# Black-Phoenix/CUDA-SfM

Hardware: AMD Instinct MI355X
Metric: RANSAC E-matrix hypotheses/sec (8-point, fused scoring), inlier-mask parity vs CPU oracle (higher is better)
Workload: dtype f32

## Files before the change

cuda-sfm_amd/csrc/ransac_prefilter.hip:

```cpp
#include "ransac_device.hpp"
#include "block_ops.hpp"
#include "prefilter_math.hpp"
#include "prefilter_record.hpp"
#include "prefilter_lds.hpp"

namespace sfm {

typedef float f16v __attribute__((ext_vector_type(16)));


__device__ constexpr int kPfESlot[9] = { 2, 6, 1, 3, 5, 7, 0, 4, 8 };
__device__ __forceinline__ uint32_t shift_in_reject(uint32_t rejected, float nt, float G)
{
    return __builtin_amdgcn_alignbit(rejected, __float_as_uint(fmaf(-nt, nt, G)), 31);
}

__device__ __forceinline__ uint32_t scan16(const f16v &nt, const f16v &G)
{
    uint32_t rejected = 0u;
#pragma unroll
    for (int r = 0; r < 16; ++r) rejected = shift_in_reject(rejected, nt[r], G[r]);
    return rejected;
}

// ... 16 lines not shown
    const uint32_t wb = pf_bfi(kPackM0 | kPackM1, pf_bfi(kPackM0, d[3], d[4]), d[5]);
    return pf_bfi(0x55555555u, wa, wb << 1);
}

typedef uint32_t u2v __attribute__((ext_vector_type(2)));
typedef float f4v __attribute__((ext_vector_type(4)));
typedef __attribute__((address_space(3))) u2v lds_u2;
typedef uint32_t u4v __attribute__((ext_vector_type(4)));
typedef __attribute__((address_space(3))) u4v lds_u4;
typedef __attribute__((address_space(3))) const f4v lds_cf4;
typedef __attribute__((address_space(3))) const float lds_cf;
typedef __attribute__((address_space(3))) int lds_i;
typedef __attribute__((address_space(3))) const h8 lds_ch8;
typedef __attribute__((address_space(3))) const v2f lds_cv2;
typedef __attribute__((address_space(3))) const unsigned char lds_cu8;

struct PfFrags { h8 n0, n1, t; };

__device__ __forceinline__ bool pf_exact_inlier(v2f p0, v2f p1, v2f p2, v2f p3, float e8, v2f xu, v2f yv, const ThrBand &band)
{
    const v2f e00 = { p3.x, p3.x }, e44 = { p3.y, p3.y }, e31 = { p1.y, p1.x };
    const v2f ab0 = __builtin_elementwise_fma(p1, yv, __builtin_elementwise_fma(e00, xu, p0));
    const v2f ab1 = __builtin_elementwise_fma(e44, yv, __builtin_elementwise_fma(e31, xu, p2));
    const float a2 = fmaf(p2.y, yv.x, fmaf(p0.y, xu.x, e8));
    const float nn = fmaf(yv.y, ab1.x, fmaf(xu.y, ab0.x, a2));
    const float n2 = nn * nn;
    const v2f dd = __builtin_elementwise_fma(ab1, ab1, ab0 * ab0);
    const float da = dd.x, db = dd.y;
    const float m = n2 * (da + db);
    const float tp = (da * db) * band.thr;
    const uint32_t mb = __float_as_uint(m), tb = __float_as_uint(tp);
    const uint32_t gap = __usad(mb, tb, 0u);
    const bool undecided = (gap < kBandUlps) || (tb < band.lo_bits) || (tb > band.hi_bits);
    bool in = m < tp;
    if (undecided) {
        const float t1 = (da == 0.0f) ? 0.0f : n2 / da;
        const float t2 = (db == 0.0f) ? 0.0f : n2 / db;
        in = (t1 + t2) < band.thr;
    }
    return in;
}

template <int RULE>
__device__ __forceinline__ PfFrags load_point_frags(lds_ch8 *frag_lane, int pb)
{
    lds_ch8 *p = frag_lane + pb * (PfLds<RULE>::kBlockBytes / 16);
    if (RULE != kPfRuleG) return PfFrags{ p[0], p[64], h8{} };
    return PfFrags{ p[0], p[64], p[128] };
}

template <int RULE>
__device__ __forceinline__ void mfma_step(const PfFrags &a, const PfFrags &b, f16v &G, f16v &nt)
{
    const f16v z = {};
    nt = __builtin_amdgcn_mfma_f32_32x32x16_f16(a.n0, b.n0, z, 0, 0, 0);
    if (RULE == kPfRuleG) G = __builtin_amdgcn_mfma_f32_32x32x16_f16(a.t, b.t, z, 0, 0, 0);
    nt = __builtin_amdgcn_mfma_f32_32x32x16_f16(a.n1, b.n1, nt, 0, 0, 0);
}

#define PF_SCHED_STEP()                                                 \
    do {                                                                \
        if (RULE != kPfRuleG) {                                         \
            __builtin_amdgcn_sched_group_barrier(0x008, 1, 0);          \
            __builtin_amdgcn_sched_group_barrier(0x002, 8, 0);          \
            __builtin_amdgcn_sched_group_barrier(0x008, 1, 0);          \
            __builtin_amdgcn_sched_group_barrier(0x002, 8, 0);          \
        } else {                                                        \
            __builtin_amdgcn_sched_group_barrier(0x008, 1, 0);          \
            __builtin_amdgcn_sched_group_barrier(0x002, 11, 0);         \
            __builtin_amdgcn_sched_group_barrier(0x008, 1, 0);          \
            __builtin_amdgcn_sched_group_barrier(0x002, 11, 0);         \
            __builtin_amdgcn_sched_group_barrier(0x008, 1, 0);          \
            __builtin_amdgcn_sched_group_barrier(0x002, 11, 0);         \
        }                                                               \
    } while (0)

constexpr int kPfVarTickets = 1;
constexpr int kPfVarDrainLocal = 2;
constexpr int kPfVarClosedDecode = 4;
constexpr int kPfVarAnswerEpilogue = 8;
constexpr int kPfVarDrainK1 = 16, kPfVarDrainK7 = 32;
constexpr int kPfVarSinglePass = 64;
constexpr int kPfVarPairDrain = 128;

constexpr int pf_score_waves_per_simd(int var, int rule, int fl2, int pipe, int wide, int prio)
{
    if ((var == 0 || var == kPfVarPairDrain) && rule == kPfRuleBandTile && !fl2 && !pipe && !wide && !prio) return 4;
    return ((var & kPfVarTickets) == 0 && (rule == kPfRuleBandTile || rule == kPfRuleBandPack) && !fl2 && !pipe && !wide && !prio) ? 5 : 4;
}

template <int W, int VAR = 0, int RULE = kPfRuleBandTile, int FL2 = 0, int PIPE = 0, int WIDE = 0, int PRIO = 0>
__global__ __launch_bounds__(W * 64, pf_score_waves_per_simd(VAR, RULE, FL2, PIPE, WIDE, PRIO))
void ransac_score_prefilter(const float *__restrict__ X0, const float *__restrict__ X1, int ld, int n,
                            const float *__restrict__ Ecand, const PfRecord *__restrict__ recs, uint32_t h0, uint32_t count, float thr,
                            int dynamic, int tile,
                            int *__restrict__ counts, uint32_t *__restrict__ tick,
                            unsigned long long *best_key, unsigned long long *best_key2, unsigned long long *__restrict__ clk,
                            const unsigned long long *__restrict__ bound_word, const uint32_t *__restrict__ tile_boxes)
{
    extern __shared__ __attribute__((aligned(16))) unsigned char smem[];
    const int lane = threadIdx.x & 63;
    const int wave = __builtin_amdgcn_readfirstlane(threadIdx.x >> 6);
    const bool probe = clk && blockIdx.x == 0 && blockIdx.y == 0 && threadIdx.x == 0;
    unsigned long long c0 = 0, w0 = 0;
    if (clk && blockIdx.x == 0 && blockIdx.y == 0 && wave == 0) { c0 = clock64(); w0 = wall_clock64(); }
#if SFM_AB
    const uint32_t trace_blk = blockIdx.y * gridDim.x + blockIdx.x;
    unsigned long long *trace = (clk && trace_blk < (uint32_t)kTraceBlocks) ? clk + 8 + (size_t)trace_blk * kTraceWords : nullptr;
    if (trace && threadIdx.x == 0) {
        trace[0] = wall_clock64();
        trace[2] = ((unsigned long long)__builtin_amdgcn_s_getreg((20 << 0) | (0 << 6) | (31 << 11)) << 32) |
                   (unsigned long long)__builtin_amdgcn_s_getreg((4 << 0) | (0 << 6) | (31 << 11));
        trace[3] = ((unsigned long long)blockIdx.y << 32) | blockIdx.x;
    }
#define PF_PHASE(k) do { if (probe1) clk[k] = wall_clock64() - w0; } while (0)
#else
#define PF_PHASE(k) do { } while (0)
#endif
    const int half = lane >> 5, row = lane & 31;
    uint32_t npass = (count + (uint32_t)kPfGroup - 1u) / (uint32_t)kPfGroup;
    const uint32_t nstatic = gridDim.x * (uint32_t)W;
    using LT = PfLds<RULE>;
    constexpr bool kBand = RULE != kPfRuleG, kTile = RULE == kPfRuleBandTile, kPack = RULE == kPfRuleBandPack || kTile;
    static_assert(!(FL2 && kPack) && !((VAR & kPfVarTickets) && kPack), "the recorded variants were built on the v_alignbit scan");
    constexpr bool kTail9 = kPack && W == 16 && !FL2 && !PIPE && !WIDE && !PRIO && !(VAR & kPfVarTickets);
    static_assert(kTail9 || (VAR & ~kPfVarTickets) == 0, "the pass-tail switches belong to the product's two rules");
    static_assert(!(VAR & kPfVarSinglePass) || (kTile && VAR == kPfVarSinglePass), "single passes: the per-tile rule's summing instance");
    static_assert(!(VAR & kPfVarPairDrain) || (kTile && VAR == kPfVarPairDrain), "paired passes drained between the scans: the per-tile rule's summing instance");
    constexpr bool kPair = kTile && kTail9 && (VAR == 0 || VAR == kPfVarPairDrain);
    constexpr bool kCarry = kPair && VAR == 0;
    constexpr int kRows = kPair ? kPfPairRows : kPfPassRows, kUnit = kRows;
    constexpr int kDrainMore = !kTail9 ? 0 : (VAR & kPfVarDrainK1) ? 1 : (VAR & kPfVarDrainK7) ? 7 : (VAR & kPfVarDrainLocal) ? 3 : 0;
    constexpr bool kDecodeTable = !(kTail9 && (VAR & kPfVarClosedDecode));
    constexpr bool kSumCounts = kTail9 && !(VAR & kPfVarAnswerEpilogue);
    constexpr int kRing = FL2 ? 256 : kPfRing;
    constexpr int kEnt = WIDE ? 16 : 8;
    static_assert(!WIDE || (kPack && !PIPE && !FL2), "wide entries: the packed scan's plain loop only");
    if (kPair) npass = (npass + 1u) >> 1;
    const LT L(tile, kRing, kEnt, kRows);
    float *etab = reinterpret_cast<float *>(smem + L.wave + wave * pf_wave_bytes(kRows));
    int *cnt = reinterpret_cast<int *>(etab + kRows * kPfERow);

    PfFrags afrag = {};
    h8 bfrag_n0 = {}, bfrag_n1 = {};
    uint32_t key0 = 0u;
    float rec_dn = 0.0f, rec_lin = 0.0f;
    float e_row[9] = {};
    auto fetch_pass = [&](uint32_t pass, PfFrags &af, uint32_t &k0, float (&e)[9], float &dn, float &lin) {
        const uint32_t hf = pass * (uint32_t)kUnit;
        const uint32_t h = hf + (uint32_t)min(kPair ? lane : row, (int)min((uint32_t)kUnit, count - hf) - 1);
        if (kTile) {
            const float *src = Ecand + 9 * (size_t)h;
#pragma unroll
            for (int k = 0; k < 9; ++k) e[k] = src[k];
            const uint4 rec = reinterpret_cast<const uint4 *>(recs)[h];
            k0 = rec.x; dn = __uint_as_float(rec.y); lin = __uint_as_float(rec.z);
            return;
        }
        const uint4 *r = reinterpret_cast<const uint4 *>(recs + h) + 2 * half;
        const uint4 r0 = r[0], r1 = r[1];
        if (kBand) pf_band_record_expand(r0, r1, half, af.n0, af.n1, k0);
        else pf_record_expand(r0, r1, half, af.n0, af.n1, af.t, k0);
        if (half == 0) {
            const float *src = Ecand + 9 * (size_t)h;
#pragma unroll
            for (int k = 0; k < 9; ++k) e[k] = src[k];
        }
    };
    auto install_rows = [&](const float (&e)[9]) {
        if (kPair || half == 0) {
            const int r = kPair ? lane : row;
#pragma unroll
            for (int k = 0; k < 9; ++k) etab[kRows * k + r] = e[kPfESlot[k]];
            cnt[r] = 0;
        }
    };
    uint32_t ps = blockIdx.x * (uint32_t)W + (uint32_t)wave;
    bool have = ps < npass;
    if (have) { fetch_pass(ps, afrag, key0, e_row, rec_dn, rec_lin); install_rows(e_row); }

    SFM_PHASE("stage_tile");
    uint32_t *next_idx = reinterpret_cast<uint32_t *>(smem + L.next);
    if (threadIdx.x == 0) *next_idx = (uint32_t)W;
    if constexpr (kCarry) {
        if (threadIdx.x < kPfRingLutBytes) smem[L.lut + threadIdx.x] = (unsigned char)pf_ring_lut_entry(threadIdx.x);
    } else
    if (kPack && kDecodeTable && threadIdx.x < 32) smem[L.lut + threadIdx.x] = (unsigned char)pf_pack_code((int)threadIdx.x);
    float pf_B = 0.0f;
    uint32_t bw[8] = {};
    uint32_t bw_lane = 0u;
    if (kTile) {
        pf_B = __uint_as_float((uint32_t)(__hip_atomic_load(reinterpret_cast<const uint32_t *>(bound_word), __ATOMIC_RELAXED, __HIP_MEMORY_SCOPE_AGENT)));
        bw_lane = __hip_atomic_load(tile_boxes + 8 * blockIdx.y + (lane & 7), __ATOMIC_RELAXED, __HIP_MEMORY_SCOPE_AGENT);
    }
    __syncthreads();
    const int tile_first = blockIdx.y * tile;
    for (int t = threadIdx.x; t < L.staged; t += W * 64) {
        const int p = tile_first + t;
        float u = 0.f, v = 0.f, x = 0.f, y = 0.f;
        const bool real = p < n && t < tile;
        if (kTile) {
            if (real) {
                const float4 q4 = reinterpret_cast<const float4 *>(X0)[p];
                u = q4.x; v = q4.y; x = q4.z; y = q4.w;
            }
        } else
        if (real) { u = X0[p]; v = X0[(size_t)ld + p]; x = X1[p]; y = X1[(size_t)ld + p]; }
        _Float16 bn[kPfSlots], bt[kPfSlotsT];
        prefilter_point_slots(u, v, x, y, real, bn, bt);
        reinterpret_cast<float4 *>(smem + L.pts)[t] = real ? make_float4(x, u, y, v) : make_float4(NAN, NAN, NAN, NAN);
        const int pb = t >> 5, col = t & 31;
        unsigned char *blk = smem + LT::kFrag + pb * LT::kBlockBytes;
#pragma unroll
        for (int ks = 0; ks < 2; ++ks)
#pragma unroll
            for (int hh = 0; hh < 2; ++hh) {
                h8 c;
#pragma unroll
                for (int j = 0; j < 8; ++j) c[j] = bn[ks * 16 + hh * 8 + j];
                *reinterpret_cast<h8 *>(blk + ks * 1024 + (hh * 32 + col) * 16) = c;
            }
        if (RULE == kPfRuleG) {
#pragma unroll
            for (int hh = 0; hh < 2; ++hh) {
                h8 c;
#pragma unroll
                for (int j = 0; j < 8; ++j) c[j] = bt[hh * 8 + j];
                *reinterpret_cast<h8 *>(blk + 2048 + (hh * 32 + col) * 16) = c;
            }
        }
    }
    __syncthreads();
    PfBox tbox = {};
    auto build_operands = [&](const float (&e)[9], uint32_t fl, float dn, float lin) {
        int half_l = half;
        float thr_l = thr, B_l = pf_B;
        asm volatile("" : "+v"(half_l), "+s"(thr_l), "+s"(B_l));
        key0 = fl & kPfTileFlagScan;
        if constexpr (kPair) {
            h8 x0, y0, x1, y1;
            pf_tile_operands_full(e, fl, dn, lin, thr_l, B_l, tbox, x0, y0, x1, y1);
            u4v xa = __builtin_bit_cast(u4v, x0), ya = __builtin_bit_cast(u4v, y0), xb = __builtin_bit_cast(u4v, x1), yb = __builtin_bit_cast(u4v, y1);
#pragma unroll
            for (int w = 0; w < 4; ++w) {
                const u2v sa = __builtin_amdgcn_permlane32_swap(xa[w], ya[w], false, false);
                const u2v sb = __builtin_amdgcn_permlane32_swap(xb[w], yb[w], false, false);
                xa[w] = sa.x; ya[w] = sa.y; xb[w] = sb.x; yb[w] = sb.y;
            }
            afrag.n0 = __builtin_bit_cast(h8, xa); afrag.n1 = __builtin_bit_cast(h8, xb);
            bfrag_n0 = __builtin_bit_cast(h8, ya); bfrag_n1 = __builtin_bit_cast(h8, yb);
        } else
        pf_tile_operands(e, fl, dn, lin, thr_l, B_l, tbox, half_l, afrag.n0, afrag.n1);
    };
    if (kTile) {
#pragma unroll
        for (int k = 0; k < 8; ++k) bw[k] = (uint32_t)__builtin_amdgcn_readlane((int)bw_lane, k);
        pf_B = uniform(pf_B);
        tbox = pf_box_from_bits(bw, pf_B);
        tbox = PfBox{ uniform(tbox.xlo), uniform(tbox.xhi), uniform(tbox.ylo), uniform(tbox.yhi), uniform(tbox.ulo), uniform(tbox.uhi), uniform(tbox.vlo), uniform(tbox.vhi) };
        if (have) build_operands(e_row, key0, rec_dn, rec_lin);
    }
#if SFM_AB
    if (probe) clk[2] = wall_clock64() - w0;
#endif
    const int npb = (min(tile, ld - tile_first) + 31) >> 5;
    const int npp = (npb + 1) >> 1;
    const float4 *pts = reinterpret_cast<const float4 *>(smem + L.pts);
    lds_cf *etab_l = (lds_cf *)etab;
    lds_i *cnt_l = (lds_i *)cnt;
    lds_cu8 *lut_l = (lds_cu8 *)(smem + L.lut);
    const uint32_t ring_base = (uint32_t)(size_t)(__attribute__((address_space(3))) unsigned char *)(smem + L.ring) + (uint32_t)wave * (uint32_t)(kRing * kEnt);
    uint32_t ring_mask = (uint32_t)(kRing * kEnt - 1);
    asm("" : "+v"(ring_mask));
    auto ring_at = [&](uint32_t index8) {
        return (lds_u2 *)((__attribute__((address_space(3))) unsigned char *)0 + ((index8 & ring_mask) | ring_base));
    };
    auto ring_at16 = [&](uint32_t index16) {
        return (lds_u4 *)((__attribute__((address_space(3))) unsigned char *)0 + ((index16 & ring_mask) | ring_base));
    };
    lds_ch8 *frag_lane = (lds_ch8 *)(smem + LT::kFrag) + lane;
    const ThrBand band = make_band(thr);
    uint32_t passes_done = 0;
#if SFM_AB
    uint32_t carried = 0;
#endif

    while (have) {
        SFM_PHASE("pass_begin");
        const uint32_t h_first = ps * (uint32_t)kUnit;
        const int nvalid_unit = (int)min((uint32_t)kUnit, count - h_first);
        int nvalid = min(nvalid_unit, kPfGroup), hoff = 0;
        const int nscan = (kPair && nvalid_unit > kPfGroup) ? 2 : 1;
#if SFM_AB
        const bool probe1 = probe && passes_done == 0u;
        unsigned long long w_scan_end = 0;
#endif
        uint32_t ps_next = ps + nstatic;
        if (dynamic) {
            uint32_t got = 0u;
            if (lane == 0) got = atomicAdd(next_idx, 1u);
            got = (uint32_t)__builtin_amdgcn_readfirstlane((int)got);
            ps_next = (got / (uint32_t)W) * nstatic + blockIdx.x * (uint32_t)W + (got % (uint32_t)W);
        }
        const unsigned long long scan_rows = __ballot(key0 != 0u);
        int head = 0, nq = 0;
        auto patch_zero_divisor_rows = [&](int sc) {
            uint32_t todo = kPair ? (uint32_t)(sc ? scan_rows >> 32 : scan_rows) : ((uint32_t)scan_rows | (uint32_t)(scan_rows >> 32));
            uint32_t survive = 0u;
            while (todo) {
                const int r = __builtin_ctz(todo) + hoff;
                todo &= todo - 1u;
                const float se[6] = { etab[6 * kRows + r], etab[2 * kRows + r], etab[r], etab[3 * kRows + r], etab[7 * kRows + r], etab[4 * kRows + r] };
                bool z = false;
                for (int j = 0; j < L.staged / 64; ++j) {
                    const float4 q = pts[j * 64 + lane];
                    z = z || prefilter_zero_divisor(se, q.x, q.z);
                }
                if (__ballot(z) != 0ull) survive |= 1u << (r - hoff);
            }
            if (survive != 0u && ((survive >> row) & 1u)) {
                const h8 zero = {};
                afrag.n0 = zero; afrag.n1 = zero; afrag.t = zero;
                if (half) { afrag.n1[3] = (_Float16)1.0f; afrag.t[7] = (_Float16)0.0009765625f; }
            }
        };

        uint32_t lane_tag = (uint32_t)(size_t)(lds_cf4 *)pts + (uint32_t)(row * 16) + (uint32_t)(half * 4);
        auto decide_first = [&](uint32_t &rest, uint32_t tag) {
            const int b = __builtin_clz(rest);
            rest &= ~(0x80000000u >> b);
            int hl, sub;
            if constexpr (kCarry) {
                const uint32_t code = (uint32_t)lut_l[pf_ring_lut_index(b, tag)];
                hl = (int)(code & 63u); sub = (int)(code >> 6);
            } else if (kPack) {
                const uint32_t code = kDecodeTable ? (uint32_t)lut_l[b] : pf_pack_code_closed(b);
                hl = (int)(code & 31u) + (int)(tag & 4u); sub = (int)(code >> 5);
            } else {
                const int r = kBand ? b >> 1 : b & 15;
                sub = kBand ? b & 1 : b >> 4;
                hl = r + (r & 12) + (int)(tag & 4u);
            }
            const int row_end = kCarry ? nvalid_unit : nvalid, row_first = kCarry ? 0 : hoff;
            if (hl < row_end) {
                const f4v q = *(lds_cf4 *)((__attribute__((address_space(3))) const unsigned char *)0 + ((tag & ~15u) + ((uint32_t)sub << 9)));
                lds_cf *e = etab_l + hl + row_first;
                const v2f p0 = { e[0], e[kRows] }, p1 = { e[2 * kRows], e[3 * kRows] }, p2 = { e[4 * kRows], e[5 * kRows] }, p3 = { e[6 * kRows], e[7 * kRows] };
                const float e8 = e[8 * kRows];
                if (pf_exact_inlier(p0, p1, p2, p3, e8, v2f{ q.x, q.y }, v2f{ q.z, q.w }, band))
                    __hip_atomic_fetch_add(cnt_l + hl + row_first, 1, __ATOMIC_RELAXED, __HIP_MEMORY_SCOPE_WORKGROUP);
            }
        };
        auto flush = [&](int m, auto more_c) {
            constexpr int kMore = decltype(more_c)::value;
            uint32_t rest = 0, tag = 0;
            if (PRIO == 2) __builtin_amdgcn_s_setprio(2);
            if (lane < m) {
                const u2v ent = *ring_at(((uint32_t)head + (uint32_t)lane) * 8u);
                tag = ent.y;
                rest = ent.x;
                decide_first(rest, tag);
                if constexpr (kMore > 0) {
#pragma unroll 1
                    for (int it = 0; it < kMore && rest != 0u; ++it) decide_first(rest, tag);
                }
            }
            const unsigned long long more = __ballot(rest != 0u);
            if (more) {
                const int slot = __builtin_amdgcn_mbcnt_hi((uint32_t)(more >> 32), __builtin_amdgcn_mbcnt_lo((uint32_t)more, 0u));
                if (rest) *ring_at(((uint32_t)(head + nq) + (uint32_t)slot) * 8u) = u2v{ rest, tag };
            }
            head = (head + m) & (kRing - 1);
            nq += __builtin_popcountll(more) - m;
            if (PRIO == 2) __builtin_amdgcn_s_setprio(0);
        };
        constexpr std::integral_constant<int, 0> kInLoop{};
        constexpr std::integral_constant<int, kDrainMore> kDrain{};
        auto flush_w = [&](int m) {
            uint32_t ra = 0, rb = 0, tag = 0;
            if (lane < m) {
                const u4v ent = *ring_at16(((uint32_t)head + (uint32_t)lane) * 16u);
                tag = ent.z;
                const bool second = ent.x == 0u;
                const uint32_t surv = second ? ent.y : ent.x;
                const int b = __builtin_clz(surv);
                const uint32_t left = surv & ~(0x80000000u >> b);
                ra = second ? 0u : left; rb = second ? left : ent.y;
                const uint32_t code = lut_l[b];
                const int hl = (int)(code & 31u) + (int)(tag & 4u);
                if (hl < nvalid) {
                    const f4v q = *(lds_cf4 *)((__attribute__((address_space(3))) const unsigned char *)0 + ((tag & ~15u) + ((code >> 5) << 9) + (second ? 1024u : 0u)));
                    lds_cf *e = etab_l + hl;
                    const v2f p0 = { e[0], e[32] }, p1 = { e[64], e[96] }, p2 = { e[128], e[160] }, p3 = { e[192], e[224] };
                    const float e8 = e[256];
                    if (pf_exact_inlier(p0, p1, p2, p3, e8, v2f{ q.x, q.y }, v2f{ q.z, q.w }, band))
                        __hip_atomic_fetch_add(cnt_l + hl, 1, __ATOMIC_RELAXED, __HIP_MEMORY_SCOPE_WORKGROUP);
                }
            }
            const unsigned long long more = __ballot((ra | rb) != 0u);
            if (more) {
                const int slot = __builtin_amdgcn_mbcnt_hi((uint32_t)(more >> 32), __builtin_amdgcn_mbcnt_lo((uint32_t)more, 0u));
                if ((ra | rb) != 0u) *ring_at16(((uint32_t)(head + nq) + (uint32_t)slot) * 16u) = u4v{ ra, rb, tag, 0u };
            }
            head = (head + m) & (kRing - 1);
            nq += __builtin_popcountll(more) - m;
        };
        auto flush2 = [&]() {
            const u2v entA = *ring_at(((uint32_t)head + (uint32_t)lane) * 8u), entB = *ring_at(((uint32_t)head + 64u + (uint32_t)lane) * 8u);
            const int bA = __builtin_clz(entA.x), bB = __builtin_clz(entB.x);
            const uint32_t restA = entA.x & ~(0x80000000u >> bA), restB = entB.x & ~(0x80000000u >> bB);
            const int rA = bA >> 1, rB = bB >> 1;
            const int hlA = rA + (rA & 12) + (int)(entA.y & 4u), hlB = rB + (rB & 12) + (int)(entB.y & 4u);
            const int hcA = min(hlA, nvalid - 1), hcB = min(hlB, nvalid - 1);
            const f4v qA = *(lds_cf4 *)((__attribute__((address_space(3))) const unsigned char *)0 + ((entA.y & ~15u) + ((uint32_t)(bA & 1) << 9)));
            const f4v qB = *(lds_cf4 *)((__attribute__((address_space(3))) const unsigned char *)0 + ((entB.y & ~15u) + ((uint32_t)(bB & 1) << 9)));
            lds_cf *eA = etab_l + hcA, *eB = etab_l + hcB;
            const v2f a0 = { eA[0], eA[32] }, a1 = { eA[64], eA[96] }, a2 = { eA[128], eA[160] }, a3 = { eA[192], eA[224] };
            const float a8 = eA[256];
            const v2f b0 = { eB[0], eB[32] }, b1 = { eB[64], eB[96] }, b2 = { eB[128], eB[160] }, b3 = { eB[192], eB[224] };
            const float b8 = eB[256];
            const bool inA = pf_exact_inlier(a0, a1, a2, a3, a8, v2f{ qA.x, qA.y }, v2f{ qA.z, qA.w }, band);
            const bool inB = pf_exact_inlier(b0, b1, b2, b3, b8, v2f{ qB.x, qB.y }, v2f{ qB.z, qB.w }, band);
            if (inA && hlA < nvalid) __hip_atomic_fetch_add(cnt_l + hlA, 1, __ATOMIC_RELAXED, __HIP_MEMORY_SCOPE_WORKGROUP);
            if (inB && hlB < nvalid) __hip_atomic_fetch_add(cnt_l + hlB, 1, __ATOMIC_RELAXED, __HIP_MEMORY_SCOPE_WORKGROUP);
            const unsigned long long moreA = __ballot(restA != 0u), moreB = __ballot(restB != 0u);
            if (moreA | moreB) {
                const int nA = __builtin_popcountll(moreA);
                const int slotA = __builtin_amdgcn_mbcnt_hi((uint32_t)(moreA >> 32), __builtin_amdgcn_mbcnt_lo((uint32_t)moreA, 0u));
                const int slotB = nA + __builtin_amdgcn_mbcnt_hi((uint32_t)(moreB >> 32), __builtin_amdgcn_mbcnt_lo((uint32_t)moreB, 0u));
                if (restA) *ring_at(((uint32_t)(head + nq) + (uint32_t)slotA) * 8u) = u2v{ restA, entA.y };
                if (restB) *ring_at(((uint32_t)(head + nq) + (uint32_t)slotB) * 8u) = u2v{ restB, entB.y };
            }
            head = (head + 128) & (kRing - 1);
            nq += __builtin_popcountll(moreA) + __builtin_popcountll(moreB) - 128;
        };

        for (int sc = 0; ; ++sc) {
        patch_zero_divisor_rows(sc);
#if SFM_AB
        if (sc == 0) PF_PHASE(3);
        else if (probe1) reinterpret_cast<uint32_t *>(clk + 3)[1] = (uint32_t)(wall_clock64() - w_scan_end);
#endif
        if constexpr (kPack && PIPE) {
        PfFrags fa = load_point_frags<RULE>(frag_lane, 0), fb = load_point_frags<RULE>(frag_lane, 1);
        lds_ch8 *fp = frag_lane + 2 * (LT::kBlockBytes / 16);
        const f16v zero16 = {};
        f16v a0, a1, b0, b1;
        a0 = __builtin_amdgcn_mfma_f32_32x32x16_f16(afrag.n0, fa.n0, zero16, 0, 0, 0);
        a1 = __builtin_amdgcn_mfma_f32_32x32x16_f16(afrag.n0, fb.n0, zero16, 0, 0, 0);
        a0 = __builtin_amdgcn_mfma_f32_32x32x16_f16(afrag.n1, fa.n1, a0, 0, 0, 0);
        a1 = __builtin_amdgcn_mfma_f32_32x32x16_f16(afrag.n1, fb.n1, a1, 0, 0, 0);
        fa = load_point_frags<RULE>(fp, 0);
        fb = load_point_frags<RULE>(fp, 1);
        fp += 2 * (LT::kBlockBytes / 16);
        auto phase = [&](const f16v &c0, const f16v &c1, f16v &m0, f16v &m1, int pp) {
            SFM_PHASE("scan_two_steps");
            __builtin_amdgcn_sched_barrier(0);
            m0 = __builtin_amdgcn_mfma_f32_32x32x16_f16(afrag.n0, fa.n0, zero16, 0, 0, 0);
            __builtin_amdgcn_sched_barrier(0);
            const u6v d = __builtin_amdgcn_cvt_scalef32_2xpk16_bf6_f32(c0, c1, 1.0f);
            __builtin_amdgcn_sched_barrier(0);
            m1 = __builtin_amdgcn_mfma_f32_32x32x16_f16(afrag.n0, fb.n0, zero16, 0, 0, 0);
            __builtin_amdgcn_sched_barrier(0);
            const uint32_t rej32 = pack_reject_bits(d);
            __builtin_amdgcn_sched_barrier(0);
            m0 = __builtin_amdgcn_mfma_f32_32x32x16_f16(afrag.n1, fa.n1, m0, 0, 0, 0);
            __builtin_amdgcn_sched_barrier(0);
            const bool mine = rej32 != 0xFFFFFFFFu;
            const unsigned long long any = __ballot(mine);
            __builtin_amdgcn_sched_barrier(0);
            m1 = __builtin_amdgcn_mfma_f32_32x32x16_f16(afrag.n1, fb.n1, m1, 0, 0, 0);
            __builtin_amdgcn_sched_barrier(0);
            fa = load_point_frags<RULE>(fp, 0);
            fb = load_point_frags<RULE>(fp, 1);
            fp += 2 * (LT::kBlockBytes / 16);
            __builtin_amdgcn_sched_barrier(0);
            SFM_PHASE("append_and_inloop_flush");
            if (any) {
                while (nq >= 64) flush(64, kInLoop);
                const int slot = __builtin_amdgcn_mbcnt_hi((uint32_t)(any >> 32), __builtin_amdgcn_mbcnt_lo((uint32_t)any, 0u));
                if (mine) *ring_at(((uint32_t)(head + nq) + (uint32_t)slot) * 8u) = u2v{ ~rej32, lane_tag + ((uint32_t)pp << 10) };
                nq += __builtin_popcountll(any);
            }
        };
        for (int pp = 0; pp < npp; pp += 2) {
            phase(a0, a1, b0, b1, pp);
            if (pp + 1 < npp) phase(b0, b1, a0, a1, pp + 1);
        }
        } else if constexpr (kPack) {
        PfFrags fa = load_point_frags<RULE>(frag_lane, 0), fb = load_point_frags<RULE>(frag_lane, 1);
        lds_ch8 *fp = frag_lane + 2 * (LT::kBlockBytes / 16);
        f16v g0, n0, n1;
        u6v dpk = {};
        auto append = [&](const u6v &d, int pp) {
            const uint32_t rej32 = pack_reject_bits(d);
            const bool mine = rej32 != 0xFFFFFFFFu;
            const unsigned long long any = __ballot(mine);
            SFM_PHASE("append_and_inloop_flush");
            if (any) {
                while (nq >= 64) flush(64, kInLoop);
                const int slot = __builtin_amdgcn_mbcnt_hi((uint32_t)(any >> 32), __builtin_amdgcn_mbcnt_lo((uint32_t)any, 0u));
                if (mine) *ring_at(((uint32_t)(head + nq) + (uint32_t)slot) * 8u) = u2v{ ~rej32, lane_tag + ((uint32_t)pp << 10) };
                nq += __builtin_popcountll(any);
            }
        };
        uint32_t rej_even = 0xFFFFFFFFu;
        auto append_w = [&](uint32_t ra, uint32_t rb, int pp_even) {
            const bool mine = (ra & rb) != 0xFFFFFFFFu;
            const unsigned long long any = __ballot(mine);
            if (any) {
                while (nq >= 64) flush_w(64);
                const int slot = __builtin_amdgcn_mbcnt_hi((uint32_t)(any >> 32), __builtin_amdgcn_mbcnt_lo((uint32_t)any, 0u));
                if (mine) *ring_at16(((uint32_t)(head + nq) + (uint32_t)slot) * 16u) = u4v{ ~ra, ~rb, lane_tag + ((uint32_t)pp_even << 10), 0u };
                nq += __builtin_popcountll(any);
            }
        };
        auto after_phase = [&](const u6v &d, int pp) {
            if (!WIDE) { append(d, pp); return; }
            const uint32_t rej32 = pack_reject_bits(d);
            if ((pp & 1) == 0) rej_even = rej32;
            else append_w(rej_even, rej32, pp - 1);
        };
        for (int pp = 0; pp < npp; ++pp) {
            SFM_PHASE("scan_two_steps");
            if (PRIO == 1) __builtin_amdgcn_s_setprio(2);
            mfma_step<RULE>(afrag, fa, g0, n0);
            mfma_step<RULE>(afrag, fb, g0, n1);
            fa = load_point_frags<RULE>(fp, 0);
            fb = load_point_frags<RULE>(fp, 1);
            fp += 2 * (LT::kBlockBytes / 16);
            if (PRIO == 1) __builtin_amdgcn_s_setprio(0);
            __builtin_amdgcn_sched_barrier(0);
            if (pp > 0) after_phase(dpk, pp - 1);
            __builtin_amdgcn_sched_barrier(0);
            dpk = __builtin_amdgcn_cvt_scalef32_2xpk16_bf6_f32(n0, n1, 1.0f);
            __builtin_amdgcn_sched_barrier(0);
        }
        after_phase(dpk, npp - 1);
        if (WIDE && (npp & 1)) append_w(rej_even, 0xFFFFFFFFu, npp - 1);
        } else {
        PfFrags fa = load_point_frags<RULE>(frag_lane, 0), fb = load_point_frags<RULE>(frag_lane, 1);
        f16v g0, n0, g1, n1;
        mfma_step<RULE>(afrag, fa, g0, n0);
        lds_ch8 *fp = frag_lane + 2 * (LT::kBlockBytes / 16);
        for (int pp = 0; pp < npp; ++pp) {
            SFM_PHASE("scan_two_steps");
            fa = load_point_frags<RULE>(fp, 0);
            __builtin_amdgcn_sched_barrier(0);
            mfma_step<RULE>(afrag, fb, g1, n1);
            const uint32_t rej_first = kBand ? scan16_band(n0) : scan16(n0, g0);
            PF_SCHED_STEP();
            __builtin_amdgcn_sched_barrier(0);
            fb = load_point_frags<RULE>(fp, 1);
            fp += 2 * (LT::kBlockBytes / 16);
            __builtin_amdgcn_sched_barrier(0);
            mfma_step<RULE>(afrag, fa, g0, n0);
            const uint32_t rej_second = kBand ? scan16_band(n1) : scan16(n1, g1);
            PF_SCHED_STEP();
            __builtin_amdgcn_sched_barrier(0);
            const uint32_t rej32 = kBand ? (((rej_first << 1) & 0xAAAAAAAAu) | (rej_second & 0x55555555u))
                                                       : ((rej_first << 16) | rej_second);
            const bool mine = rej32 != 0xFFFFFFFFu;
            const unsigned long long any = __ballot(mine);
            SFM_PHASE("append_and_inloop_flush");
            if (any) {
                if (FL2) { while (nq >= 128) flush2(); }
                else
                while (nq >= 64) flush(64, kInLoop);
                const int slot = __builtin_amdgcn_mbcnt_hi((uint32_t)(any >> 32), __builtin_amdgcn_mbcnt_lo((uint32_t)any, 0u));
                if (mine) *ring_at(((uint32_t)(head + nq) + (uint32_t)slot) * 8u) = u2v{ ~rej32, lane_tag + ((uint32_t)pp << 10) };
                nq += __builtin_popcountll(any);
            }
        }
        }
        if (sc + 1 >= nscan) break;
#if SFM_AB
        if (probe1) w_scan_end = wall_clock64();
#endif
        if constexpr (kCarry) lane_tag |= kPfTagScan;
        else while (nq > 0) flush(min(nq, 64), kDrain);
#if SFM_AB
        carried += (uint32_t)nq;
#endif
        afrag.n0 = bfrag_n0; afrag.n1 = bfrag_n1;
        hoff = kPfGroup; nvalid = nvalid_unit - kPfGroup;
        }
        PF_PHASE(4);
        SFM_PHASE("pass_end_fetch_next");
        const bool have_next = ps_next < npass;
        PfFrags afrag_next = afrag;
        uint32_t key0n = 0u;
        float e_next[9] = {}, dn_next = 0.0f, lin_next = 0.0f;
        if (have_next) fetch_pass(ps_next, afrag_next, key0n, e_next, dn_next, lin_next);
        SFM_PHASE("drain_flush");
        if (FL2) { while (nq >= 128) flush2(); }
        if (WIDE) { while (nq > 0) flush_w(min(nq, 64)); }
        while (nq > 0) flush(min(nq, 64), kDrain);
        SFM_PHASE("epilogue");
        PF_PHASE(7);
        if (VAR & kPfVarTickets) {
        if (lane < nvalid) {
            const int c = cnt[lane];
            if (c) atomicAdd(&counts[h_first + lane], c);
        }
        asm volatile("s_waitcnt vmcnt(0)" ::: "memory");
        uint32_t t = 0;
        if (lane == 0) t = atomicAdd(&tick[ps], 1u);
        t = __builtin_amdgcn_readfirstlane(t);
        if (t == gridDim.y - 1) {
            unsigned long long k = 0;
            if (lane < nvalid) {
                const int c = __hip_atomic_load(&counts[h_first + lane], __ATOMIC_RELAXED, __HIP_MEMORY_SCOPE_AGENT);
                k = pack_key((uint32_t)c, h0 + h_first + (uint32_t)lane);
            }
            k = wave_max(k);
            if (lane == 0 && k) {
                atomicMax(best_key, k);
                if (best_key2) atomicMax(best_key2, k);
            }
        }
        } else if (kSumCounts) {
        if (lane < nvalid_unit) {
// ... 379 lines not shown
        prefilter_transposed(e, et);
        out[100] = (float)prefilter_zero_divisor_cells(et, B, prefilter_grid(B), cx0, cx1, cy0, cy1);
    }
    {
        const int j = (lane & 31) >> 1, st = lane & 1;
        f16v s0, s1;
#pragma unroll
        for (int k = 0; k < 16; ++k) { s0[k] = (k == j && st == 0) ? u : 256.0f; s1[k] = (k == j && st == 1) ? u : 256.0f; }
        const uint32_t surv = ~pack_reject_bits(__builtin_amdgcn_cvt_scalef32_2xpk16_bf6_f32(s0, s1, 1.0f));
        bool ok;
        if (prefilter_band_pack_reject(u)) ok = surv == 0u;
        else {
            const int b = __builtin_clz(surv | 1u);
            ok = surv != 0u && (surv & (surv - 1u)) == 0u && pf_pack_code(b) == ((uint32_t)((j & 3) + 8 * (j >> 2)) | ((uint32_t)st << 5));
        }
        const unsigned long long okm = __ballot(ok && lane < 32);
        if (lane == 0) { out[101] = (float)__builtin_popcountll(okm); out[102] = (float)(surv == 0u); }
    }
}

int launch_prefilter_band_probe(sfm_ctx *ctx, const float *d_E, float thr, float B, const float box[8], int b_safe, const float pt[4], int survive_all, float *d_out)
{
    const PfBox bx = { box[0], box[1], box[2], box[3], box[4], box[5], box[6], box[7] };
    hipLaunchKernelGGL(pf_band_probe_kernel, dim3(1), dim3(64), 0, ctx->stream, d_E, thr, B, bx, b_safe, pt[0], pt[1], pt[2], pt[3], survive_all,
                       reinterpret_cast<PfRecord *>(d_out + 128), d_out);
    SFM_HIP_TRY(hipGetLastError());
    return SFM_OK;
}

int launch_prefilter_probe(sfm_ctx *ctx, const float *d_E, float thr, float B, const float pt[4], int survive_all, float *d_out)
{
    PfScales sc;
    if (!prefilter_scales(thr, sc)) { set_error("threshold %g outside the pre-filter's range", (double)thr); return SFM_E_INVALID; }
    hipLaunchKernelGGL(pf_probe_kernel, dim3(1), dim3(64), 0, ctx->stream, d_E, thr, B, sc, pt[0], pt[1], pt[2], pt[3], survive_all,
                       reinterpret_cast<PfRecord *>(d_out + 128), d_out);
    SFM_HIP_TRY(hipGetLastError());
    return SFM_OK;
}
#endif

static int pf_rule_switch(const sfm_ransac_params &p)
{
    if (SFM_SW(p, 3) == 4 || SFM_SW(p, 3) >= 16) return kPfRuleG;
    if (SFM_SW(p, 3) == 5 || SFM_SW(p, 1) == 5 || SFM_SW(p, 1) == 7 || SFM_SW(p, 1) == 9) return kPfRuleBand;
    if (SFM_SW(p, 3) == 6 || SFM_SW(p, 1) == 11 || SFM_SW(p, 1) == 12) return kPfRuleBandPack;
    if (SFM_SW(p, 3) == 7 || SFM_SW(p, 1) == 13 || SFM_SW(p, 1) == 14 || SFM_SW(p, 1) == 15) return kPfRuleBandTile;
    return -1;
}

constexpr uint64_t kPfOrderFirstCallPairs = 1ull << 33;
int prefilter_pick_rule(sfm_pair *pair, const sfm_ransac_params &p, uint32_t count)
{
    int rule = pf_rule_switch(p);
    if (rule < 0) {
        const bool ordered = pair->sorted_epoch == pair->bound_epoch && pair->d_pts4s != nullptr;
        const bool first = pair->pf_seen_epoch != pair->bound_epoch;
        rule = (!ordered && first && (uint64_t)count * (uint64_t)pair->ld < kPfOrderFirstCallPairs) ? kPfRuleBandPack : kPfRuleBandTile;
    }
    pair->pf_seen_epoch = pair->bound_epoch;
    pair->pf_rule = rule;
    return rule;
}

bool prefilter_usable(const sfm_pair *pair, const sfm_ransac_params &p, uint32_t count)
{
    PfScales sc;
    return pair->state.unit_z && pair->state.have_bound && count >= 16384u && (uint64_t)count * (uint64_t)pair->ld >= (1ull << 27) && prefilter_scales(p.threshold, sc);
}

static int pf_tile_of(const sfm_pair *pair, const sfm_ransac_params &p)
{
    if (SFM_SW(p, 1) == 7 && pair->pf_rule == kPfRuleBand) return pf_tile_points(pair->ld, 1536);
    return pf_tile_points(pair->ld, kPfTileMax);
}

int prefilter_tile_points(const sfm_pair *pair, const sfm_ransac_params &p) { return pf_tile_of(pair, p); }

static int pf_tail_var(const sfm_pair *pair, const sfm_ransac_params &p, uint32_t count)
{
    const bool large = pf_sums_counts_at(count, pair->ld, pf_tile_of(pair, p));
    if (SFM_SW(p, 1) == 19) return 0;
    if (SFM_SW(p, 1) == 20) return pair->pf_rule == kPfRuleBandTile ? kPfVarSinglePass : 0;
    if (SFM_SW(p, 1) == 21) return pair->pf_rule == kPfRuleBandTile ? kPfVarPairDrain : 0;
    if (pair->pf_rule == kPfRuleBandTile && SFM_SW(p, 1) == 16) return kPfVarDrainK1;
    if (pair->pf_rule == kPfRuleBandTile && SFM_SW(p, 1) == 17) return kPfVarDrainK7;
    int var = 0;
    const bool lab = SFM_SW(p, 3) >= 8 && SFM_SW(p, 3) < 16;
    if (lab && (SFM_SW(p, 3) & 1)) var |= kPfVarDrainLocal;
    if (lab && (SFM_SW(p, 3) & 2)) var |= kPfVarClosedDecode;
    const bool sum = (lab && (SFM_SW(p, 3) & 4)) ? false : (large || (SFM_SW(p, 1) >= 16 && SFM_SW(p, 1) <= 18));
    if (!sum) var |= kPfVarAnswerEpilogue;
    if (var == 0 && pair->pf_rule == kPfRuleBandTile && !pf_pairs_passes_at(count, pair->ld, pf_tile_of(pair, p))) var = kPfVarSinglePass;
    return var;
}

bool prefilter_sums_counts(const sfm_pair *pair, const sfm_ransac_params &p, uint32_t count)
{
    const bool product_rule = pair->pf_rule == kPfRuleBandTile || pair->pf_rule == kPfRuleBandPack;
    const bool variant = SFM_SW(p, 1) == 5 || (SFM_SW(p, 1) >= 11 && SFM_SW(p, 1) <= 15);
    return product_rule && !variant && !(pf_tail_var(pair, p, count) & kPfVarAnswerEpilogue);
}

int launch_score_prefilter(sfm_pair *pair, ShardSlot &s, hipStream_t stream, const sfm_ransac_params &p, uint32_t h0, uint32_t count, unsigned long long *key2)
{
    sfm_ctx *ctx = pair->ctx;
    PfScales sc;
    if (!prefilter_scales(p.threshold, sc)) { set_error("threshold %g outside the pre-filter's range", (double)p.threshold); return SFM_E_INVALID; }
    const int waves = (SFM_SW(p, 1) == 5 || SFM_SW(p, 1) == 12) ? 12 : kPfWaves;
    const int tile = pf_tile_of(pair, p);
    const int ntiles = (pair->ld + tile - 1) / tile;
    const uint32_t npass = (count + (uint32_t)kPfGroup - 1u) / (uint32_t)kPfGroup;
    const int rule = pair->pf_rule;
    const int tail_var = pf_tail_var(pair, p, count);
    const bool wide = rule == kPfRuleBandTile && SFM_SW(p, 1) == 13;
    const bool paired_units = rule == kPfRuleBandTile && (tail_var == 0 || tail_var == kPfVarPairDrain) && waves == kPfWaves && !wide && SFM_SW(p, 1) != 14 && SFM_SW(p, 1) != 15;
    const uint32_t nunits = paired_units ? (npass + 1u) / 2u : npass;
    const uint32_t iters = (nunits + (uint32_t)waves - 1) / (uint32_t)waves;
    uint32_t cols = (uint32_t)ctx->num_cus / (uint32_t)ntiles;
    if (SFM_SW(p, 2) > 0) cols = (uint32_t)SFM_SW(p, 2);
    if (cols > iters) cols = iters;
    if (cols < 1) cols = 1;
    const int dynamic = SFM_SW(p, 1) == 2 ? 0 : 1;
    const int var = SFM_SW(p, 3) >= 16 ? SFM_SW(p, 3) - 16 : 0;
    const bool fl2 = rule == kPfRuleBand && waves == kPfWaves && SFM_SW(p, 1) == 9;
    const int lds_bytes = wide ? PfLds<kPfRuleBand>(tile, kPfRing, 16, kPfPassRows).bytes : fl2 ? PfLds<kPfRuleBand>(tile, 256, 8, kPfPassRows).bytes
                        : rule != kPfRuleG ? PfLds<kPfRuleBand>(tile, kPfRing, 8, paired_units ? kPfPairRows : kPfPassRows).bytes : PfLds<kPfRuleG>(tile).bytes;
    if (lds_bytes > 160 * 1024) { set_error("pre-filter tile of %d points needs %d bytes of LDS", tile, lds_bytes); return SFM_E_INVALID; }
    auto launch = [&](auto kernel) -> int {
        const int rc_lds = allow_big_lds(ctx, reinterpret_cast<const void *>(kernel));
        if (rc_lds != SFM_OK) return rc_lds;
        const float *x0 = rule == kPfRuleBandTile ? reinterpret_cast<const float *>(pair->d_pts4s) : pair->d_X[0];
        hipLaunchKernelGGL(kernel, dim3(cols, ntiles), dim3(waves * 64), lds_bytes, stream,
                           x0, pair->d_X[1], pair->ld, pair->n, s.Ecand, reinterpret_cast<const PfRecord *>(s.pf), h0, count, p.threshold,
                           dynamic, tile, s.counts, s.tick, s.key, key2, pair->d_clk, pair->d_bound, pair->d_tile_boxes);
        return SFM_OK;
    };
    int rcl;
#if SFM_AB
    if (rule == kPfRuleG && waves == 12) rcl = launch(&ransac_score_prefilter<12, 0, kPfRuleG>);
    else if (rule == kPfRuleG && var == 1) rcl = launch(&ransac_score_prefilter<16, 1, kPfRuleG>);
    else if (rule == kPfRuleG) rcl = launch(&ransac_score_prefilter<16, 0, kPfRuleG>);
    else if (waves == 12) rcl = launch(&ransac_score_prefilter<12, 0, kPfRuleBand>);
    else if (fl2) rcl = launch(&ransac_score_prefilter<16, 0, kPfRuleBand, 1>);
    else if (rule == kPfRuleBand) rcl = launch(&ransac_score_prefilter<16, 0, kPfRuleBand>);
    else if (SFM_SW(p, 1) == 11) rcl = launch(&ransac_score_prefilter<16, 0, kPfRuleBandPack, 0, 1>);
    else if (SFM_SW(p, 1) == 12) rcl = launch(&ransac_score_prefilter<12, 0, kPfRuleBandPack, 0, 1>);
    else if (wide) rcl = launch(&ransac_score_prefilter<16, 0, kPfRuleBandTile, 0, 0, 1>);
    else if (rule == kPfRuleBandTile && SFM_SW(p, 1) == 14) rcl = launch(&ransac_score_prefilter<16, 0, kPfRuleBandTile, 0, 0, 0, 1>);
    else if (rule == kPfRuleBandTile && SFM_SW(p, 1) == 15) rcl = launch(&ransac_score_prefilter<16, 0, kPfRuleBandTile, 0, 0, 0, 2>);
    else if (tail_var != 0 && tail_var != kPfVarAnswerEpilogue && tail_var != kPfVarSinglePass) {
        rcl = SFM_E_INVALID;
#define PF_TAIL_CASE(V) case V: rcl = rule == kPfRuleBandPack ? launch(&ransac_score_prefilter<16, V, kPfRuleBandPack>) : launch(&ransac_score_prefilter<16, V, kPfRuleBandTile>); break
        switch (tail_var) {
        PF_TAIL_CASE(2); PF_TAIL_CASE(4); PF_TAIL_CASE(6); PF_TAIL_CASE(10); PF_TAIL_CASE(12); PF_TAIL_CASE(14);
        case kPfVarDrainK1: rcl = launch(&ransac_score_prefilter<16, kPfVarDrainK1, kPfRuleBandTile>); break;
        case kPfVarDrainK7: rcl = launch(&ransac_score_prefilter<16, kPfVarDrainK7, kPfRuleBandTile>); break;
        case kPfVarPairDrain: rcl = launch(&ransac_score_prefilter<16, kPfVarPairDrain, kPfRuleBandTile>); break;
        default: set_error("pass-tail switches %d: no such instance", tail_var); break;
        }
#undef PF_TAIL_CASE
    }
    else
#endif
    if (tail_var & kPfVarAnswerEpilogue) rcl = rule == kPfRuleBandPack ? launch(&ransac_score_prefilter<16, kPfVarAnswerEpilogue, kPfRuleBandPack>)
                                                                       : launch(&ransac_score_prefilter<16, kPfVarAnswerEpilogue, kPfRuleBandTile>);
    else if (rule == kPfRuleBandPack) rcl = launch(&ransac_score_prefilter<16, 0, kPfRuleBandPack>);
    else if (tail_var == kPfVarSinglePass) rcl = launch(&ransac_score_prefilter<16, kPfVarSinglePass, kPfRuleBandTile>);
    else rcl = launch(&ransac_score_prefilter<16, 0, kPfRuleBandTile>);
    (void)var; (void)fl2; (void)wide; (void)tail_var;
    if (rcl != SFM_OK) return rcl;
    SFM_HIP_TRY(hipGetLastError());
    pair->last_grid = (int)cols * ntiles; pair->last_block = waves * 64; pair->last_lds = lds_bytes;
    return SFM_OK;
}

}
```

Baseline: 2.936 billion.

## Interleave the two paired-pass scans in one point walk sharing fragment loads

In the default paired-pass instance (VAR 0), the two hypothesis groups are now scanned together in a single walk over the point fragments. Each loaded point fragment feeds MFMAs for both the first group (afrag) and the second group (bfrag), and reject entries are tagged by scan. Before, each group made its own pass over the points. The old back-to-back behaviour is kept as a new switch-selected variant (PairSeq). The aim is to halve point-fragment LDS loads and overlap the two scans' MFMA and append work. In exchange it adds register pressure and requires the drain code to handle scan-tagged ring entries.

```diff
diff --git a/cuda-sfm_amd/csrc/ransac_prefilter.hip b/cuda-sfm_amd/csrc/ransac_prefilter.hip
--- a/cuda-sfm_amd/csrc/ransac_prefilter.hip
+++ b/cuda-sfm_amd/csrc/ransac_prefilter.hip
@@ -122,10 +122,11 @@
 constexpr int kPfVarDrainK1 = 16, kPfVarDrainK7 = 32;
 constexpr int kPfVarSinglePass = 64;
 constexpr int kPfVarPairDrain = 128;
+constexpr int kPfVarPairSeq = 256;
 
 constexpr int pf_score_waves_per_simd(int var, int rule, int fl2, int pipe, int wide, int prio)
 {
-    if ((var == 0 || var == kPfVarPairDrain) && rule == kPfRuleBandTile && !fl2 && !pipe && !wide && !prio) return 4;
+    if ((var == 0 || var == kPfVarPairDrain || var == kPfVarPairSeq) && rule == kPfRuleBandTile && !fl2 && !pipe && !wide && !prio) return 4;
     return ((var & kPfVarTickets) == 0 && (rule == kPfRuleBandTile || rule == kPfRuleBandPack) && !fl2 && !pipe && !wide && !prio) ? 5 : 4;
 }
 
@@ -167,8 +168,10 @@
     static_assert(kTail9 || (VAR & ~kPfVarTickets) == 0, "the pass-tail switches belong to the product's two rules");
     static_assert(!(VAR & kPfVarSinglePass) || (kTile && VAR == kPfVarSinglePass), "single passes: the per-tile rule's summing instance");
     static_assert(!(VAR & kPfVarPairDrain) || (kTile && VAR == kPfVarPairDrain), "paired passes drained between the scans: the per-tile rule's summing instance");
-    constexpr bool kPair = kTile && kTail9 && (VAR == 0 || VAR == kPfVarPairDrain);
-    constexpr bool kCarry = kPair && VAR == 0;
+    static_assert(!(VAR & kPfVarPairSeq) || (kTile && VAR == kPfVarPairSeq), "paired passes scanned back to back: the per-tile rule's summing instance");
+    constexpr bool kPair = kTile && kTail9 && (VAR == 0 || VAR == kPfVarPairDrain || VAR == kPfVarPairSeq);
+    constexpr bool kCarry = kPair && VAR != kPfVarPairDrain;
+    constexpr bool kInter = kPair && VAR == 0;
     constexpr int kRows = kPair ? kPfPairRows : kPfPassRows, kUnit = kRows;
     constexpr int kDrainMore = !kTail9 ? 0 : (VAR & kPfVarDrainK1) ? 1 : (VAR & kPfVarDrainK7) ? 7 : (VAR & kPfVarDrainLocal) ? 3 : 0;
     constexpr bool kDecodeTable = !(kTail9 && (VAR & kPfVarClosedDecode));
@@ -330,7 +333,8 @@
         const uint32_t h_first = ps * (uint32_t)kUnit;
         const int nvalid_unit = (int)min((uint32_t)kUnit, count - h_first);
         int nvalid = min(nvalid_unit, kPfGroup), hoff = 0;
-        const int nscan = (kPair && nvalid_unit > kPfGroup) ? 2 : 1;
+        const bool two_scans = kPair && nvalid_unit > kPfGroup;
+        const int nscan = (two_scans && !kInter) ? 2 : 1;
 #if SFM_AB
         const bool probe1 = probe && passes_done == 0u;
         unsigned long long w_scan_end = 0;
@@ -347,8 +351,9 @@
         auto patch_zero_divisor_rows = [&](int sc) {
             uint32_t todo = kPair ? (uint32_t)(sc ? scan_rows >> 32 : scan_rows) : ((uint32_t)scan_rows | (uint32_t)(scan_rows >> 32));
             uint32_t survive = 0u;
+            const int row0 = kInter ? kPfGroup * sc : hoff;
             while (todo) {
-                const int r = __builtin_ctz(todo) + hoff;
+                const int r = __builtin_ctz(todo) + row0;
                 todo &= todo - 1u;
                 const float se[6] = { etab[6 * kRows + r], etab[2 * kRows + r], etab[r], etab[3 * kRows + r], etab[7 * kRows + r], etab[4 * kRows + r] };
                 bool z = false;
@@ -356,12 +361,17 @@
                     const float4 q = pts[j * 64 + lane];
                     z = z || prefilter_zero_divisor(se, q.x, q.z);
                 }
-                if (__ballot(z) != 0ull) survive |= 1u << (r - hoff);
+                if (__ballot(z) != 0ull) survive |= 1u << (r - row0);
             }
             if (survive != 0u && ((survive >> row) & 1u)) {
                 const h8 zero = {};
+                if (kInter && sc) {
+                    bfrag_n0 = zero; bfrag_n1 = zero;
+                    if (half) bfrag_n1[3] = (_Float16)1.0f;
+                } else {
                 afrag.n0 = zero; afrag.n1 = zero; afrag.t = zero;
                 if (half) { afrag.n1[3] = (_Float16)1.0f; afrag.t[7] = (_Float16)0.0009765625f; }
+                }
             }
         };
 
@@ -477,6 +487,9 @@
 
         for (int sc = 0; ; ++sc) {
         patch_zero_divisor_rows(sc);
+        if constexpr (kInter) {
+            if (two_scans) patch_zero_divisor_rows(1);
+        }
 #if SFM_AB
         if (sc == 0) PF_PHASE(3);
         else if (probe1) reinterpret_cast<uint32_t *>(clk + 3)[1] = (uint32_t)(wall_clock64() - w_scan_end);
@@ -528,11 +541,11 @@
             if (pp + 1 < npp) phase(b0, b1, a0, a1, pp + 1);
         }
         } else if constexpr (kPack) {
-        PfFrags fa = load_point_frags<RULE>(frag_lane, 0), fb = load_point_frags<RULE>(frag_lane, 1);
+        PfFrags fa = kInter ? PfFrags{} : load_point_frags<RULE>(frag_lane, 0), fb = kInter ? PfFrags{} : load_point_frags<RULE>(frag_lane, 1);
         lds_ch8 *fp = frag_lane + 2 * (LT::kBlockBytes / 16);
         f16v g0, n0, n1;
         u6v dpk = {};
-        auto append = [&](const u6v &d, int pp) {
+        auto append = [&](const u6v &d, int pp, uint32_t scan_tag) {
             const uint32_t rej32 = pack_reject_bits(d);
             const bool mine = rej32 != 0xFFFFFFFFu;
             const unsigned long long any = __ballot(mine);
@@ -540,7 +553,7 @@
             if (any) {
                 while (nq >= 64) flush(64, kInLoop);
                 const int slot = __builtin_amdgcn_mbcnt_hi((uint32_t)(any >> 32), __builtin_amdgcn_mbcnt_lo((uint32_t)any, 0u));
-                if (mine) *ring_at(((uint32_t)(head + nq) + (uint32_t)slot) * 8u) = u2v{ ~rej32, lane_tag + ((uint32_t)pp << 10) };
+                if (mine) *ring_at(((uint32_t)(head + nq) + (uint32_t)slot) * 8u) = u2v{ ~rej32, lane_tag + (((uint32_t)pp << 10) | scan_tag) };
                 nq += __builtin_popcountll(any);
             }
         };
@@ -556,11 +569,54 @@
             }
         };
         auto after_phase = [&](const u6v &d, int pp) {
-            if (!WIDE) { append(d, pp); return; }
+            if (!WIDE) { append(d, pp, 0u); return; }
             const uint32_t rej32 = pack_reject_bits(d);
             if ((pp & 1) == 0) rej_even = rej32;
             else append_w(rej_even, rej32, pp - 1);
         };
+        bool walked = false;
+        if constexpr (kInter) {
+        if (two_scans) {
+            const PfFrags bfrag = { bfrag_n0, bfrag_n1, h8{} };
+            lds_ch8 *fl = frag_lane;
+            asm("" : "+v"(fl));
+            fa = load_point_frags<RULE>(fl, 0); fb = load_point_frags<RULE>(fl, 1);
+            fp = fl + 2 * (LT::kBlockBytes / 16);
+            for (int pp = 0; pp < npp; ++pp) {
+                SFM_PHASE("scan_two_steps");
+                mfma_step<RULE>(afrag, fa, g0, n0);
+                mfma_step<RULE>(afrag, fb, g0, n1);
+                __builtin_amdgcn_sched_barrier(0);
+                if (pp > 0) {
+#if SFM_AB
+                    carried += (uint32_t)nq;
+#endif
+                    append(dpk, pp - 1, kPfTagScan);
+                }
+                __builtin_amdgcn_sched_barrier(0);
+                dpk = __builtin_amdgcn_cvt_scalef32_2xpk16_bf6_f32(n0, n1, 1.0f);
+                __builtin_amdgcn_sched_barrier(0);
+                SFM_PHASE("scan_two_steps");
+                mfma_step<RULE>(bfrag, fa, g0, n0);
+                mfma_step<RULE>(bfrag, fb, g0, n1);
+                fa = load_point_frags<RULE>(fp, 0);
+                fb = load_point_frags<RULE>(fp, 1);
+                fp += 2 * (LT::kBlockBytes / 16);
+                __builtin_amdgcn_sched_barrier(0);
+                append(dpk, pp, 0u);
+                __builtin_amdgcn_sched_barrier(0);
+                dpk = __builtin_amdgcn_cvt_scalef32_2xpk16_bf6_f32(n0, n1, 1.0f);
+                __builtin_amdgcn_sched_barrier(0);
+            }
+#if SFM_AB
+            carried += (uint32_t)nq;
+#endif
+            append(dpk, npp - 1, kPfTagScan);
+            walked = true;
+        }
+        }
+        if (!walked) {
+        if constexpr (kInter) { fa = load_point_frags<RULE>(frag_lane, 0); fb = load_point_frags<RULE>(frag_lane, 1); }
         for (int pp = 0; pp < npp; ++pp) {
             SFM_PHASE("scan_two_steps");
             if (PRIO == 1) __builtin_amdgcn_s_setprio(2);
@@ -578,6 +634,7 @@
         }
         after_phase(dpk, npp - 1);
         if (WIDE && (npp & 1)) append_w(rej_even, 0xFFFFFFFFu, npp - 1);
+        }
         } else {
         PfFrags fa = load_point_frags<RULE>(frag_lane, 0), fb = load_point_frags<RULE>(frag_lane, 1);
         f16v g0, n0, g1, n1;
@@ -1123,6 +1180,7 @@
     if (SFM_SW(p, 1) == 19) return 0;
     if (SFM_SW(p, 1) == 20) return pair->pf_rule == kPfRuleBandTile ? kPfVarSinglePass : 0;
     if (SFM_SW(p, 1) == 21) return pair->pf_rule == kPfRuleBandTile ? kPfVarPairDrain : 0;
+    if (SFM_SW(p, 1) == 22) return pair->pf_rule == kPfRuleBandTile ? kPfVarPairSeq : 0;
     if (pair->pf_rule == kPfRuleBandTile && SFM_SW(p, 1) == 16) return kPfVarDrainK1;
     if (pair->pf_rule == kPfRuleBandTile && SFM_SW(p, 1) == 17) return kPfVarDrainK7;
     int var = 0;
@@ -1154,7 +1212,7 @@
     const int rule = pair->pf_rule;
     const int tail_var = pf_tail_var(pair, p, count);
     const bool wide = rule == kPfRuleBandTile && SFM_SW(p, 1) == 13;
-    const bool paired_units = rule == kPfRuleBandTile && (tail_var == 0 || tail_var == kPfVarPairDrain) && waves == kPfWaves && !wide && SFM_SW(p, 1) != 14 && SFM_SW(p, 1) != 15;
+    const bool paired_units = rule == kPfRuleBandTile && (tail_var == 0 || tail_var == kPfVarPairDrain || tail_var == kPfVarPairSeq) && waves == kPfWaves && !wide && SFM_SW(p, 1) != 14 && SFM_SW(p, 1) != 15;
     const uint32_t nunits = paired_units ? (npass + 1u) / 2u : npass;
     const uint32_t iters = (nunits + (uint32_t)waves - 1) / (uint32_t)waves;
     uint32_t cols = (uint32_t)ctx->num_cus / (uint32_t)ntiles;
@@ -1197,6 +1255,7 @@
         case kPfVarDrainK1: rcl = launch(&ransac_score_prefilter<16, kPfVarDrainK1, kPfRuleBandTile>); break;
         case kPfVarDrainK7: rcl = launch(&ransac_score_prefilter<16, kPfVarDrainK7, kPfRuleBandTile>); break;
         case kPfVarPairDrain: rcl = launch(&ransac_score_prefilter<16, kPfVarPairDrain, kPfRuleBandTile>); break;
+        case kPfVarPairSeq: rcl = launch(&ransac_score_prefilter<16, kPfVarPairSeq, kPfRuleBandTile>); break;
         default: set_error("pass-tail switches %d: no such instance", tail_var); break;
         }
 #undef PF_TAIL_CASE
```

After: 3.029 billion, median of 6. 1.03x the previous value.
